# AlessioSam/LADiff

Hardware: AMD Instinct MI355X
Metric: motions/sec (196-frame, 50-step DDIM, bs128) (higher is better)
Workload: dtype f16x3+f32; 1 GPU; headline:ddim50_cfg7.5_b128_f196_c263_humanml3d; prompts_per_gpu=128, global_batch=128, frames=196, scheduler=ddim, denoising_steps=50, parallelism=dp1, loop=persistent pipeline kernel (16-row blocks x 86)

## Files before the change

### include/ladiff_hip_debug.h

```cpp
#ifndef LADIFF_HIP_DEBUG_H
#define LADIFF_HIP_DEBUG_H

#include "ladiff_hip.h"

#ifdef __cplusplus
extern "C" {
#endif

LADIFF_API int ladiff_debug_set_stage_waves(int waves_per_simd);
LADIFF_API int ladiff_debug_set_handoff(int tagged);
LADIFF_API int ladiff_debug_set_stage_plan(int v);
LADIFF_API int ladiff_debug_set_poll_pause(int mask, int len);
LADIFF_API int ladiff_debug_set_stage_delay(int mask, int len);
LADIFF_API int ladiff_debug_set_pacing(int eighths, int mask);
LADIFF_API int ladiff_debug_set_xcd_local(int on);
LADIFF_API int ladiff_debug_set_decoder_fusion(int on);
LADIFF_API int ladiff_debug_set_mlp_variant(int v);

LADIFF_API int ladiff_debug_set_loop_thresholds(int look_ahead_from, int small_upto);
LADIFF_API int ladiff_debug_set_graph_epoch_rule(int on);
LADIFF_API int ladiff_debug_graph_instantiations(void);

#ifdef LADIFF_STAMPS
LADIFF_API void ladiff_debug_set_stamps(unsigned long long* p);
LADIFF_API void ladiff_debug_set_sys_stamps(unsigned long long* p);
LADIFF_API void ladiff_debug_set_probe(int v);
#endif

#ifdef __cplusplus
}
#endif
#endif
```

### ladiff_amd/_lib.py

```python
import ctypes
import os
from ctypes import c_char_p, c_double, c_float, c_int, c_size_t, c_uint64, c_void_p

import numpy as np
import torch

_HERE = os.path.dirname(os.path.abspath(__file__))
LIB_PATH = os.path.join(_HERE, "libladiff_hip.so")

MAX_LATENTS = 8
MAX_FRAMES = 224
COEF_STRIDE = 8
COEF_K_NOISE, COEF_K_M = 5, 6
ACT = {"none": 0, "relu": 1, "gelu": 2, "silu": 3, "qgelu": 4, "lrelu": 5}


class LadiffHipError(RuntimeError):
    pass


SPLIT_MODES = ("f16x3", "bf16x3", "split")


def is_split(precision):
# ... 72 lines not shown
    "ladiff_debug_set_stage_delay": (c_int, [c_int, c_int]),
    "ladiff_debug_set_pacing": (c_int, [c_int, c_int]),
    "ladiff_debug_set_loop_thresholds": (c_int, [c_int, c_int]),
    "ladiff_debug_set_graph_epoch_rule": (c_int, [c_int]),
    "ladiff_debug_graph_instantiations": (c_int, []),
    "ladiff_sampler_set_fault": (c_int, [c_void_p, c_int, c_int]),
    "ladiff_sampler_set_noise_generator": (c_int, [c_void_p, c_uint64, ctypes.c_uint32, c_int]),
    "ladiff_noise_fill": (c_int, [c_uint64, ctypes.c_uint32, c_int, c_int, c_int, c_int, c_void_p, c_void_p]),
    "ladiff_reverse_workspace_bytes": (c_size_t, [c_int, c_int, c_int, c_int]),
    "ladiff_diffusion_reverse": (c_int, [c_void_p, c_void_p, c_void_p, c_uint64, c_void_p, c_void_p, c_void_p, c_void_p, c_void_p,
                                         c_void_p, c_void_p, c_void_p, c_float, c_float, c_int, c_int, c_int, c_int, c_int,
                                         c_void_p, c_void_p, c_size_t, c_int, c_void_p]),
    "ladiff_diffusion_reverse_prompts": (c_int, [c_void_p, c_void_p, c_void_p, c_uint64, c_void_p, c_void_p, c_void_p, c_void_p, c_void_p,
                                                 c_void_p, c_void_p, c_void_p, c_float, c_float, c_int, c_int, c_int, c_int, c_int,
                                                 c_void_p, c_void_p, c_size_t, c_int, c_void_p, c_void_p, c_void_p, c_int, c_void_p]),
    "ladiff_diffusion_reverse_multistep": (c_int, [c_void_p, c_void_p, c_void_p, c_uint64, c_void_p, c_void_p, c_void_p, c_void_p, c_void_p,
                                                   c_void_p, c_void_p, c_void_p, c_float, c_float, c_int, c_int, c_int, c_int, c_int,
                                                   c_void_p, c_void_p, c_size_t, c_int, c_void_p, c_void_p, c_void_p, c_int, c_void_p,
                                                   c_void_p]),
    "ladiff_diffusion_reverse_from": (c_int, [c_void_p, c_void_p, c_void_p, c_uint64, c_void_p, c_void_p, c_void_p, c_void_p, c_void_p,
                                              c_void_p, c_void_p, c_void_p, c_float, c_float, c_int, c_int, c_int, c_int, c_int,
                                              c_void_p, c_void_p, c_size_t, c_int, c_void_p, c_void_p, c_void_p, c_int, c_void_p,
                                              c_void_p, c_void_p, c_int, c_void_p]),
    "ladiff_diffusion_reverse_record": (c_int, [c_void_p, c_void_p, c_void_p, c_uint64, c_void_p, c_void_p, c_void_p, c_void_p, c_void_p,
                                                c_void_p, c_void_p, c_void_p, c_float, c_float, c_int, c_int, c_int, c_int, c_int,
                                                c_void_p, c_void_p, c_size_t, c_int, c_void_p, c_void_p, c_void_p, c_int, c_void_p,
                                                c_void_p, c_void_p, c_int, c_void_p, c_void_p, c_void_p]),
    "ladiff_noise_fill_prompts": (c_int, [c_void_p, c_void_p, c_int, c_int, c_int, c_int, c_void_p, c_void_p]),
    "ladiff_encoder_num_params": (c_int, []),
    "ladiff_encoder_param_name": (c_char_p, [c_int]),
    "ladiff_encoder_workspace_bytes": (c_size_t, [c_int, c_int, c_int, c_int]),
    "ladiff_vae_encode": (c_int, [c_void_p, c_void_p, c_void_p, c_void_p, c_void_p, c_void_p, c_int, c_int, c_int, c_int,
                                  c_void_p, c_void_p, c_void_p, c_void_p, c_size_t, c_void_p]),
    "ladiff_vae_encode_dvae": (c_int, [c_void_p, c_void_p, c_void_p, c_void_p, c_void_p, c_void_p, c_int, c_int, c_int, c_int,
                                       c_void_p, c_void_p, c_void_p, c_void_p, c_size_t, c_void_p, c_void_p, c_int, c_void_p]),
    "ladiff_vae_losses_workspace_bytes": (c_size_t, [c_int, c_int, c_int, c_int, c_int]),
    "ladiff_vae_losses": (c_int, [c_void_p, c_void_p, c_void_p, c_void_p, c_void_p, c_void_p, c_int, c_int, c_int, c_int, c_int,
                                  c_double, c_double, c_double, c_void_p, c_void_p, c_void_p, c_size_t, c_void_p]),
    "ladiff_denoiser_forward_timesteps_workspace_bytes": (c_size_t, [c_int, c_int]),
    "ladiff_denoiser_forward_timesteps": (c_int, [c_void_p, c_void_p, c_void_p, c_int, c_void_p, c_void_p, c_int, c_int, c_void_p, c_void_p,
                                                  c_void_p, c_size_t, c_void_p]),
    "ladiff_q_sample": (c_int, [c_void_p, c_void_p, c_void_p, c_int, c_void_p, c_int, c_uint64, ctypes.c_uint32, c_void_p, c_void_p, c_int,
                                c_int, c_void_p]),
    "ladiff_diffusion_losses_workspace_bytes": (c_size_t, [ctypes.c_int64]),
    "ladiff_diffusion_losses": (c_int, [c_void_p, c_void_p, ctypes.c_int64, c_double, c_void_p, c_void_p, c_void_p, c_size_t, c_void_p]),
    "ladiff_clip_num_params": (c_int, []),
    "ladiff_clip_param_name": (c_char_p, [c_int]),
    "ladiff_clip_workspace_bytes": (c_size_t, [c_int, c_int]),
    "ladiff_clip_text_encode": (c_int, [c_void_p, c_void_p, c_int, c_int, c_void_p, c_int, c_int, c_int, c_void_p, c_void_p,
                                        c_size_t, c_void_p]),
    "ladiff_clip_workspace_bytes_ragged": (c_size_t, [c_int, c_int]),
    "ladiff_clip_text_encode_ragged": (c_int, [c_void_p, c_void_p, c_int, c_int, c_void_p, c_int, c_int, c_int, c_void_p, c_void_p,
                                               c_void_p, c_int, c_void_p, c_void_p, c_size_t, c_void_p]),
    "ladiff_t2m_movement_num_params": (c_int, []),
    "ladiff_t2m_movement_param_name": (c_char_p, [c_int]),
    "ladiff_t2m_motion_num_params": (c_int, []),
    "ladiff_t2m_motion_param_name": (c_char_p, [c_int]),
    "ladiff_t2m_text_num_params": (c_int, []),
    "ladiff_t2m_text_param_name": (c_char_p, [c_int]),
    "ladiff_t2m_movement_workspace_bytes": (c_size_t, [c_int, c_int, c_int]),
    "ladiff_t2m_motion_workspace_bytes": (c_size_t, [c_int, c_int]),
    "ladiff_t2m_text_workspace_bytes": (c_size_t, [c_int, c_int]),
    "ladiff_t2m_movement_encode": (c_int, [c_void_p, c_void_p, c_int, c_int, c_int, c_int, c_void_p, c_void_p, c_size_t,
                                           c_void_p]),
    "ladiff_t2m_motion_encode": (c_int, [c_void_p, c_void_p, c_void_p, c_int, c_int, c_void_p, c_void_p, c_size_t, c_void_p]),
    "ladiff_t2m_text_encode": (c_int, [c_void_p, c_void_p, c_void_p, c_void_p, c_int, c_int, c_void_p, c_void_p, c_size_t,
                                       c_void_p]),
    "ladiff_feats2joints": (c_int, [c_void_p, c_void_p, c_void_p, c_int, c_int, c_int, c_int, c_void_p, c_void_p]),
    "ladiff_joints2feats": (c_int, [c_void_p, c_void_p, c_int, c_int, c_int, c_void_p, c_float, c_void_p, c_void_p, c_void_p, c_void_p]),
    "ladiff_joint_ape_ave": (c_int, [c_void_p, c_void_p, c_void_p, c_void_p, c_int, c_int, c_int, c_void_p, c_float, c_void_p, c_void_p,
                                     c_void_p]),
    "ladiff_joint_mr": (c_int, [c_void_p, c_void_p, c_void_p, c_int, c_int, c_int, c_void_p, c_void_p, c_void_p]),
    "ladiff_render_workspace_bytes": (c_size_t, [c_int]),
    "ladiff_render_motion": (c_int, [c_void_p, c_void_p, c_int, c_int, c_int, c_void_p, c_int, c_int, c_int, c_int, c_void_p, c_int, c_void_p,
                                     c_size_t, c_void_p]),
    "ladiff_decoder_workspace_bytes": (c_size_t, [c_int, c_int, c_int, c_int]),
    "ladiff_vae_decode": (c_int, [c_void_p, c_void_p, c_void_p, c_void_p, c_void_p, c_int, c_int, c_int, c_int, c_void_p,
                                  c_void_p, c_size_t, c_void_p]),
    "ladiff_debug_set_stage_waves": (c_int, [c_int]),
    "ladiff_debug_set_handoff": (c_int, [c_int]),
    "ladiff_debug_set_xcd_local": (c_int, [c_int]),
    "ladiff_debug_set_decoder_fusion": (c_int, [c_int]),
    "ladiff_debug_set_mlp_variant": (c_int, [c_int]),
    "ladiff_reverse_plan": (c_int, [c_int, c_int, c_void_p, c_int, c_int, c_int, c_int, c_void_p, c_void_p]),
    "ladiff_decoder_graph_create": (c_int, [ctypes.POINTER(c_void_p)]),
    "ladiff_decoder_graph_destroy": (c_int, [c_void_p]),
    "ladiff_vae_decode_graphed": (c_int, [c_void_p, c_void_p, c_void_p, c_uint64, c_void_p, c_void_p, c_void_p, c_void_p, c_int, c_int, c_int,
                                          c_int, c_int, c_void_p, c_void_p, c_size_t, c_void_p]),
    "ladiff_vae_decode_ragged": (c_int, [c_void_p, c_void_p, c_void_p, c_void_p, c_void_p, c_void_p, c_int, c_int, c_int, c_int,
                                         c_int, c_void_p, c_void_p, c_size_t, c_void_p]),
    "ladiff_vae_decode_att_maps": (c_int, [c_void_p, c_void_p, c_void_p, c_void_p, c_void_p, c_void_p, c_int, c_int, c_int, c_int,
                                           c_int, c_void_p, c_void_p, c_void_p, c_size_t, c_void_p]),
}

EXPORTS = tuple(_SIGNATURES)
_lib = None
LIB_PATH_BF16 = os.path.join(_HERE, "libladiff_hip_bf16.so")


def select_split_format(fmt):
    global LIB_PATH, _lib
    if fmt not in ("fp16", "bf16"):
        raise ValueError(f'split format must be "fp16" or "bf16", got {fmt!r}')
    path = LIB_PATH_BF16 if fmt == "bf16" else os.path.join(_HERE, "libladiff_hip.so")
    if _lib is not None and path != LIB_PATH:
        raise LadiffHipError("select_split_format() after the library has been used: weight tables of the other format exist")
    LIB_PATH = path


def lib():
    global _lib
    if _lib is None:
        if not os.path.exists(LIB_PATH):
            raise LadiffHipError(f"{LIB_PATH} not found: build it with `python -m ladiff_amd.build` "
                                 "(the HIP library is the only implementation of this path; there is no CPU fallback)")
        cdll = ctypes.CDLL(LIB_PATH)
        for name, (res, args) in _SIGNATURES.items():
            fn = getattr(cdll, name)
            fn.restype, fn.argtypes = res, args
        _lib = cdll
    return _lib


def check(rc):
    if rc != 0:
        raise LadiffHipError(f"libladiff_hip: {lib().ladiff_error_string(rc).decode()} (code {rc})")


def ptr(t, dtype=torch.float32):
    if t is None:
        return None
    if not t.is_cuda:
        raise LadiffHipError("libladiff_hip works on GPU tensors only; got a CPU tensor (no CPU fallback exists)")
    if t.dtype != dtype:
        raise LadiffHipError(f"expected {dtype}, got {t.dtype}")
    if not t.is_contiguous():
        raise LadiffHipError("expected a contiguous tensor")
    return t.data_ptr()


def stream_ptr():
    return torch.cuda.current_stream().cuda_stream


def param_names(kind):
    l = lib()
    n = getattr(l, f"ladiff_{kind}_num_params")()
    return [getattr(l, f"ladiff_{kind}_param_name")(i).decode() for i in range(n)]


class WeightTable:
    _next_generation = 1

    def __init__(self, kind, tensors, n_names=None, no_split=(), pad_rows=None):
        self.generation = WeightTable._next_generation
        WeightTable._next_generation += 1
        names = param_names(kind)
        if n_names is not None:
            names = names[:n_names]
        self.no_split = set(no_split)
        self.pad_rows = dict(pad_rows or {})
        self.names = names
        self.tensors = []
        for n in names:
            if n not in tensors:
                raise LadiffHipError(f"missing weight {n}")
# ... 107 lines not shown
```

### ladiff_amd/build.py

```python
import os
import subprocess
import sys
from concurrent.futures import ThreadPoolExecutor

HERE = os.path.dirname(os.path.abspath(__file__))
CSRC = os.path.join(HERE, "csrc")
OBJ = os.path.join(HERE, "csrc", "build")
LIB = os.path.join(HERE, "libladiff_hip.so")
SOURCES = ["gemm.hip", "gemm_big.hip", "gemm_kr.hip", "gemm_rowln.hip", "rowops.hip", "attention.hip", "qkv_attn.hip", "systolic.hip", "systolic_plan.hip", "linear_ca.hip", "dec_cross.hip", "dec_mlp.hip", "dec_post.hip", "dec_qkv_attn.hip", "feats2joints.hip", "joints2feats.hip", "joint_metrics.hip", "render.hip", "vae_losses.hip", "denoiser.hip", "diffusion_stage.hip", "decoder.hip", "encoder.hip", "clip.hip", "evaluator.hip", "reverse.hip", "api.hip"]
FLAGS = ["--offload-arch=gfx950", "-O3", "-std=c++17", "-fPIC", "-fvisibility=hidden", "-Wall", "-Wno-unused-function"]


def _hipcc():
    for c in (os.environ.get("HIPCC"), "/opt/rocm/bin/hipcc", "hipcc"):
        if c and (os.path.isabs(c) and os.path.exists(c) or not os.path.isabs(c)):
            return c
    raise RuntimeError("hipcc not found")


def _stale(target, deps):
    if not os.path.exists(target):
        return True
    t = os.path.getmtime(target)
    return any(os.path.getmtime(d) > t for d in deps)


def stamps_lib(level=1):
    return LIB.replace(".so", "_stamps.so" if int(level) == 1 else f"_stamps{int(level)}.so")


def diag_lib():
    return LIB.replace(".so", "_diag.so")


def build(force=False, verbose=False, stamps=False, tag=None, defines=(), only=None):
    obj, lib, flags = OBJ, LIB, list(FLAGS)
    if tag:
        obj, lib = OBJ + "_" + tag, LIB.replace(".so", f"_{tag}.so")
        flags += ["-D" + d for d in defines]
    if stamps:
        lvl = os.environ.get("LADIFF_STAMPS_LEVEL", "1")
        obj, lib = OBJ + "_stamps" + (lvl if lvl != "1" else ""), stamps_lib(lvl)
        flags.append("-DLADIFF_STAMPS=" + lvl)
    os.makedirs(obj, exist_ok=True)
    headers = [os.path.join(CSRC, f) for f in os.listdir(CSRC) if f.endswith(".h")]
    headers += [os.path.join(os.path.dirname(HERE), "include", h) for h in ("ladiff_hip.h", "ladiff_hip_debug.h")]
    hipcc = _hipcc()
    jobs = []
    objdir = {src: (obj if only is None or src in only else OBJ) for src in SOURCES}
    for src in SOURCES:
        s = os.path.join(CSRC, src)
        o = os.path.join(objdir[src], src.replace(".hip", ".o"))
        if objdir[src] == obj and (force or _stale(o, [s] + headers)):
            jobs.append([hipcc, *flags, "-c", s, "-o", o])

    def run(cmd):
        if verbose:
            print(" ".join(cmd), flush=True)
        r = subprocess.run(cmd, capture_output=True, text=True)
        if r.returncode != 0:
            raise RuntimeError(f"hipcc failed: {' '.join(cmd)}\n{r.stdout}\n{r.stderr}")
        return r.stderr

    with ThreadPoolExecutor(max_workers=4) as ex:
        for err in ex.map(run, jobs):
            if verbose and err.strip():
                print(err)
    objs = [os.path.join(objdir[s], s.replace(".hip", ".o")) for s in SOURCES]
    if force or jobs or _stale(lib, objs + [os.path.join(CSRC, "exports.map")]):
        run([hipcc, "--offload-arch=gfx950", "-shared", "-fPIC", "-fvisibility=hidden", "-Wl,--version-script=" + os.path.join(CSRC, "exports.map"),
             "-o", lib, *objs])
    return lib


def build_all(force=False, verbose=False):
    lib = build(force=force, verbose=verbose)
    build(force=force, verbose=verbose, tag="bf16", defines=["LADIFF_SPLIT_BF16"])
    build(force=force, verbose=verbose, tag="diag", defines=["LADIFF_TAG_BITS=4", "LADIFF_SELFCHECK"], only=("systolic.hip",))
    return lib


if __name__ == "__main__":
    _tag = next((a.split("=", 1)[1] for a in sys.argv if a.startswith("--tag=")), None)
    _defs = [a[2:] for a in sys.argv if a.startswith("-D")]
    if "--all" in sys.argv:
        print(build_all(force="--force" in sys.argv, verbose=True))
    else:
        print(build(force="--force" in sys.argv, verbose=True, stamps="--stamps" in sys.argv, tag=_tag, defines=_defs))
```

### ladiff_amd/csrc/api.hip

```cpp
#include <algorithm>
#include <cstdlib>
#include <cstring>
#include <vector>

#include "model.h"
#include "sampler.h"
#include "../../include/ladiff_hip_debug.h"

using namespace ladiff;

namespace {

inline hipStream_t S(ladiff_stream_t s) { return reinterpret_cast<hipStream_t>(s); }

bool all_set(const float* const* w, size_t n) {
    if (w == nullptr) return false;
    for (size_t i = 0; i < n; ++i)
        if (w[i] == nullptr) return false;
    return true;
}
template <class W>
bool load_weights(W& dst, const float* const* ptrs) {
    if (!all_set(ptrs, sizeof(W) / sizeof(const float*))) return false;
    std::memcpy(&dst, ptrs, sizeof(W));
// ... 207 lines not shown
int ladiff_init_latents(const float* noise, const int32_t* counts, float sigma, float* latents, int B, int T,
                        ladiff_stream_t stream) {
    LADIFF_CHECK_ARG(noise && latents && B > 0 && T > 0);
    return launch_init_latents(noise, counts, sigma, latents, B, T, S(stream));
}
int ladiff_init_latents_from(const float* z0, const float* noise, const uint64_t* seeds, const uint32_t* prompt_index, const int32_t* counts,
                             const float* coef, const int32_t* starts, int first_step, float* latents, int B, int T, ladiff_stream_t stream) {
    LADIFF_CHECK_ARG(z0 && coef && latents && B > 0 && T > 0 && first_step >= 0);
    LADIFF_CHECK_ARG(noise != nullptr || seeds != nullptr);
    LADIFF_CHECK_ARG(prompt_index == nullptr || seeds != nullptr);
    if ((reinterpret_cast<uintptr_t>(z0) & 15) || (reinterpret_cast<uintptr_t>(noise) & 15) || (reinterpret_cast<uintptr_t>(latents) & 15) ||
        (reinterpret_cast<uintptr_t>(seeds) & 7) || (reinterpret_cast<uintptr_t>(prompt_index) & 3) || (reinterpret_cast<uintptr_t>(starts) & 3))
        return LADIFF_ERR_SHAPE;
    const NoiseGen gen = noise == nullptr ? NoiseGen{0u, 0u, 0u, 1, reinterpret_cast<const unsigned long long*>(seeds), prompt_index}
                                          : NoiseGen{0u, 0u, 0u, 0};
    return launch_init_latents_from(z0, noise, gen, counts, coef, starts, first_step, latents, B, T, nullptr, S(stream));
}
int ladiff_finalize_latents(const float* latents, const int32_t* counts, float* z, int B, int T, ladiff_stream_t stream) {
    LADIFF_CHECK_ARG(latents && z && B > 0 && T > 0);
    return launch_finalize_latents(latents, counts, z, B, T, S(stream));
}

int ladiff_sampler_create(void** sampler) {
    LADIFF_CHECK_ARG(sampler);
    *sampler = new Sampler();
    return 0;
}
int ladiff_sampler_destroy(void* sampler) {
    Sampler* sp = reinterpret_cast<Sampler*>(sampler);
    if (sp == nullptr) return 0;
    (void)hipDeviceSynchronize();
    sp->drain_retired();
    if (sp->exec) (void)hipGraphExecDestroy(sp->exec);
    if (sp->setup) (void)hipGraphExecDestroy(sp->setup);
    if (sp->ev0) (void)hipEventDestroy(sp->ev0);
    if (sp->ev1) (void)hipEventDestroy(sp->ev1);
    for (hipEvent_t e : sp->wev) (void)hipEventDestroy(e);
    sp->cap.destroy();
    delete sp;
    return 0;
}

int ladiff_reverse_plan(int B, int T, const int32_t* h_counts, int masked, int loop_mode, int f16x3, int cfg, int* rows_per_block, int* n_blocks) {
    LADIFF_CHECK_ARG(B >= 1 && T >= 1 && T <= LADIFF_MAX_LATENTS && loop_mode >= 1 && loop_mode <= 3 && rows_per_block && n_blocks);
    if (!cfg && masked && h_counts == nullptr) return LADIFF_ERR_UNSUPPORTED;
    std::vector<unsigned char> plan;
    int mr = 2, nb = 0;
    choose_plan(B, T, h_counts, masked != 0, loop_mode, f16x3 != 0, plan, &mr, &nb, cfg != 0);
    *rows_per_block = 16 * mr; *n_blocks = nb;
    return 0;
}

int ladiff_debug_set_stage_waves(int waves_per_simd) {
    LADIFF_CHECK_ARG(waves_per_simd == 1 || waves_per_simd == 2);
    g_loop.waves16 = waves_per_simd;
    return 0;
}

int ladiff_debug_set_handoff(int tagged) {
    LADIFF_CHECK_ARG(tagged == 0 || tagged == 1);
    g_loop.handoff = tagged;
    return 0;
}

int ladiff_debug_set_mlp_variant(int v) {
#ifdef LADIFF_STAMPS
    LADIFF_CHECK_ARG((v >= 0 && v <= 3) || (v >= 11 && v <= 17) || (v >= 21 && v <= 26));
#else
    LADIFF_CHECK_ARG(v >= 0 && v <= 3);
#endif
    g_dec.mlp_variant = v;
    return 0;
}

int ladiff_debug_set_decoder_fusion(int on) {
    LADIFF_CHECK_ARG(on >= 0 && on <= 254 && (on & 3) != 3 && (on & 48) != 48);
    g_dec.post_off = (on & 128) ? 1 : 0;
    g_dec.out_cross = (on & 64) ? 0 : 1;
    g_dec.fused_mlp = on & 3;
    g_dec.small_rows_path = (on & 4) ? 0 : 1;
    g_dec.final_split = (on & 8) ? 0 : 1;
    g_dec.fused_attn = (on & 16) ? 0 : (on & 32) ? 2 : 1;
    return 0;
}

int ladiff_debug_set_stage_plan(int v) {
    LADIFF_CHECK_ARG(v >= 0 && v <= 1);
    g_loop.stage_plan = v;
    return 0;
}

int ladiff_debug_set_poll_pause(int mask, int len) {
    LADIFF_CHECK_ARG(mask >= 0 && mask <= 255 && len >= 0 && len <= 64);
    g_loop.poll_pause = mask | (len << 8);
    return 0;
}

int ladiff_debug_set_pacing(int eighths, int mask) {
    if (eighths == -1) { g_loop.pace = -1; return 0; }
    LADIFF_CHECK_ARG(eighths >= 0 && eighths <= 8 && mask >= 0 && mask <= 255);
    g_loop.pace = eighths | (mask << 8);
    return 0;
}

int ladiff_debug_set_stage_delay(int mask, int len) {
    LADIFF_CHECK_ARG(mask >= -1 && mask <= 255 && len >= 0 && len <= 64);
    g_loop.stage_delay = mask < 0 ? -1 : (mask | (len << 8));
    return 0;
}

int ladiff_debug_set_loop_thresholds(int look_ahead_from, int small_upto) {
    LADIFF_CHECK_ARG(look_ahead_from >= -1 && small_upto >= -1);
    g_loop.look_ahead_from = look_ahead_from;
    g_loop.small_upto = small_upto;
    return 0;
}

int ladiff_debug_set_graph_epoch_rule(int on) {
    LADIFF_CHECK_ARG(on == 0 || on == 1);
    g_graph_epoch_rule = on;
    return 0;
}

int ladiff_debug_graph_instantiations(void) { return g_graph_instantiations.load(); }

int ladiff_debug_set_xcd_local(int on) {
    LADIFF_CHECK_ARG(on >= 0 && on <= 2);
    g_loop.xcd_local = on;
    return 0;
}

int ladiff_sampler_set_loop(void* sampler, int mode) {
    Sampler* sp = reinterpret_cast<Sampler*>(sampler);
    LADIFF_CHECK_ARG(sp != nullptr && mode >= 0 && mode <= 3);
    sp->loop = mode != 0;
    sp->loop_mode = mode;
    return 0;
}

int ladiff_sampler_loop_ms(void* sampler, float* ms) {
    Sampler* sp = reinterpret_cast<Sampler*>(sampler);
    LADIFF_CHECK_ARG(sp != nullptr && ms != nullptr && sp->ev1 != nullptr);
    LADIFF_HIP(hipEventSynchronize(sp->ev1));
    LADIFF_HIP(hipEventElapsedTime(ms, sp->ev0, sp->ev1));
    return 0;
}

int ladiff_sampler_set_window_timing(void* sampler, int on) {
    Sampler* sp = reinterpret_cast<Sampler*>(sampler);
    LADIFF_CHECK_ARG(sp != nullptr);
    sp->time_windows = on != 0;
    return 0;
}

int ladiff_sampler_window_ms(void* sampler, float* loop_ms_sum, int* n_windows) {
    Sampler* sp = reinterpret_cast<Sampler*>(sampler);
    LADIFF_CHECK_ARG(sp != nullptr && loop_ms_sum != nullptr && n_windows != nullptr);
    float sum = 0.f;
    for (int i = 0; i < sp->n_windows; ++i) {
        float ms = 0.f;
        LADIFF_HIP(hipEventSynchronize(sp->wev[2 * i + 1]));
        LADIFF_HIP(hipEventElapsedTime(&ms, sp->wev[2 * i], sp->wev[2 * i + 1]));
        sum += ms;
    }
    *loop_ms_sum = sum; *n_windows = sp->n_windows;
    return 0;
// ... 487 lines not shown
```

### ladiff_amd/csrc/denoiser.hip

```cpp
#include "model.h"

namespace ladiff {

static std::vector<std::string> block_prefixes(const char* root) {
    std::vector<std::string> v;
    for (int i = 0; i < NSKIP; ++i) v.push_back(std::string(root) + ".input_blocks." + std::to_string(i));
    v.push_back(std::string(root) + ".middle_block");
    for (int i = 0; i < NSKIP; ++i) v.push_back(std::string(root) + ".output_blocks." + std::to_string(i));
    return v;
}
static void wb(std::vector<std::string>& v, const std::string& p) { v.push_back(p + ".weight"); v.push_back(p + ".bias"); }
static void mha_names(std::vector<std::string>& v, const std::string& p) {
    v.push_back(p + ".in_proj_weight"); v.push_back(p + ".in_proj_bias"); wb(v, p + ".out_proj");
}
static void styl_names(std::vector<std::string>& v, const std::string& p) {
    wb(v, p + ".emb_layers.1"); wb(v, p + ".norm"); wb(v, p + ".out_layers.2");
}

const std::vector<std::string>& denoiser_param_names() {
    static const std::vector<std::string> names = [] {
        std::vector<std::string> v;
        wb(v, "time_embedding.linear_1"); wb(v, "time_embedding.linear_2"); wb(v, "emb_proj.1");
        v.push_back("query_pos.pe"); v.push_back("mem_pos.pe");
        wb(v, "encoder.norm");
// ... 27 lines not shown
        return v;
    }();
    return names;
}

const std::vector<std::string>& encoder_param_names() {
    static const std::vector<std::string> names = [] {
        std::vector<std::string> v;
        v.push_back("global_motion_token"); v.push_back("query_pos_encoder.pe");
        for (const auto& p : block_prefixes("encoder")) {
            mha_names(v, p + ".self_attn");
            wb(v, p + ".linear1"); wb(v, p + ".linear2");
            wb(v, p + ".norm1"); wb(v, p + ".norm2");
        }
        for (int i = 0; i < NSKIP; ++i) wb(v, "encoder.linear_blocks." + std::to_string(i));
        wb(v, "encoder.norm"); wb(v, "skel_embedding");
        return v;
    }();
    return names;
}

int denoiser_time_tables(const DenoiserW& w, const float* sinus, int n, float* tables, float* ws, size_t ws_floats,
                         hipStream_t s) {
    const DenTimeWs t = den_time_layout(ws, n);
    if (ws_floats < t.total) return LADIFF_ERR_WORKSPACE;
    float *h1 = t.h1, *temb = t.temb, *semb = t.semb;
    LADIFF_TRY(launch_gemm(lin(sinus, TEXT_DIM, w.time1, h1, D, n, D, TEXT_DIM, ACT_SILU), s));
    LADIFF_TRY(launch_gemm(lin(h1, D, w.time2, temb, D, n, D, D), s));
    LADIFF_TRY(launch_silu(temb, semb, (size_t)n * D, s));
    for (int l = 0; l < NL; ++l) {
        const DenLayerW& L = w.layer[l];
        float* base = tables + (size_t)l * DEN_LAYER_STRIDE;
        LADIFF_TRY(launch_gemm(lin(semb, D, L.ca_proj.emb, base + DEN_OFF_CA_MOD, DEN_STEP_STRIDE, n, 2 * D, D), s));
        LADIFF_TRY(launch_gemm(lin(semb, D, L.ffn_proj.emb, base + DEN_OFF_FFN_MOD, DEN_STEP_STRIDE, n, 2 * D, D), s));
        LinearW kvw{L.sa_attn.in_w + (size_t)D * D, L.sa_attn.in_b + D};
        LADIFF_TRY(launch_gemm(lin(temb, D, kvw, base + DEN_OFF_TIME_KV, DEN_STEP_STRIDE, n, 2 * D, D), s));
    }
    return 0;
}

static int denoiser_text_cache_general(const DenoiserW& w, const float* text, int B2, int N, float* cache, float* ws, size_t ws_floats,
                                       hipStream_t s) {
    const int R = B2 * N;
    const DenTextWs t = den_text_layout(ws, B2, 1, N);
    if (ws_floats < t.total) return LADIFF_ERR_WORKSPACE;
    const DenTextCache c = den_text_cache_layout(cache, B2, 1, N);
    float *rl = t.rl, *tn = t.tn, *key = t.key, *val = t.val, *tproj = c.tproj, *tkv = c.tkv, *catt = c.catt;
    LADIFF_TRY(launch_relu(text, rl, (size_t)R * TEXT_DIM, s));
    LADIFF_TRY(launch_gemm(lin(rl, TEXT_DIM, w.emb_proj, tproj, D, R, D, TEXT_DIM), s));
    for (int l = 0; l < NL; ++l) {
        const DenLayerW& L = w.layer[l];
        LinearW kvw{L.sa_attn.in_w + (size_t)D * D, L.sa_attn.in_b + D};
        LADIFF_TRY(launch_gemm(lin(tproj, D, kvw, tkv + (size_t)l * R * 2 * D, 2 * D, R, 2 * D, D), s));
        LADIFF_TRY(launch_layernorm(tproj, L.ca_text_norm.g, L.ca_text_norm.b, tn, R, s));
        LADIFF_TRY(launch_gemm(lin(tn, D, L.ca_key, key, D, R, D, D), s));
        LADIFF_TRY(launch_gemm(lin(tn, D, L.ca_value, val, D, R, D, D), s));
        LADIFF_TRY(launch_lca_kv(key, val, B2, N, catt + (size_t)l * B2 * H * DH * DH, s));
    }
    return 0;
}

int denoiser_text_static(const DenoiserW& w, const float* text, int B2, float* cache, float* ws, size_t ws_floats, hipStream_t s) {
    const DenTextWs t = den_text_layout(ws, B2, 0, 1);
    if (ws_floats < t.total) return LADIFF_ERR_WORKSPACE;
    const DenTextCache c = den_text_cache_layout(cache, B2, 0, 1);
    float *rl = t.rl, *tn = t.tn, *tproj = c.tproj, *tkv = c.tkv, *nval = c.nval;
    LADIFF_TRY(launch_relu(text, rl, (size_t)B2 * TEXT_DIM, s));
    LADIFF_TRY(launch_gemm(lin(rl, TEXT_DIM, w.emb_proj, tproj, D, B2, D, TEXT_DIM), s));
    GemmArgs kv[NL], val[NL];
    RowBatch ln;
    for (int l = 0; l < NL; ++l) {
        const DenLayerW& L = w.layer[l];
        LinearW kvw{L.sa_attn.in_w + (size_t)D * D, L.sa_attn.in_b + D};
        kv[l] = lin(tproj, D, kvw, tkv + (size_t)l * B2 * 2 * D, 2 * D, B2, 2 * D, D);
        ln.a[l] = tproj; ln.g[l] = L.ca_text_norm.g; ln.b[l] = L.ca_text_norm.b; ln.y[l] = tn + (size_t)l * B2 * D;
        val[l] = lin(tn + (size_t)l * B2 * D, D, L.ca_value, nval + (size_t)l * B2 * D, D, B2, D, D);
        val[l].ln_g = L.ca_proj.norm.g; val[l].ln_b = L.ca_proj.norm.b;
    }
    LADIFF_TRY(launch_gemm_batch(kv, NL, s));
    LADIFF_TRY(launch_layernorm_batch(ln, NL, B2, s));
    return launch_gemm_batch(val, NL, s);
}

int denoiser_ctab(const DenoiserW& w, const float* tables_lo, int n, float* cache, int B2, float* u, size_t u_floats, hipStream_t s,
                  const DenoiserW* wsp) {
    const int R = B2 + 1;
    const size_t u_all = den_text_layout(nullptr, B2, n, 1).u_floats;
    if (u_floats < u_all / NL) return LADIFF_ERR_WORKSPACE;
    const DenTextCache c = den_text_cache_layout(cache, B2, n, 1);
    const float* nval = c.nval;
    float* ctab = c.ctab;
    if (u_floats >= u_all) {
        RowBatch rb;
        GemmArgs g[NL];
        for (int l = 0; l < NL; ++l) {
            const DenLayerW& L = w.layer[l];
            float* ul = u + (size_t)l * n * R * D;
            rb.a[l] = nval + (size_t)l * B2 * D; rb.g[l] = L.ca_proj.norm.b;
            rb.b[l] = tables_lo + (size_t)l * DEN_LAYER_STRIDE + DEN_OFF_CA_MOD; rb.y[l] = ul;
            g[l] = lin(ul, D, L.ca_proj.out, ctab + (size_t)l * n * R * D, D, n * R, D, D);
            if (wsp != nullptr) { g[l].W = wsp->layer[l].ca_proj.out.w; g[l].split = 1; }
        }
        LADIFF_TRY(launch_ca_table_input_batch(rb, NL, DEN_STEP_STRIDE, n, B2, s, wsp != nullptr ? 1 : 0));
        return launch_gemm_batch(g, NL, s);
    }
    for (int l = 0; l < NL; ++l) {
        const DenLayerW& L = w.layer[l];
        LADIFF_TRY(launch_ca_table_input(nval + (size_t)l * B2 * D, L.ca_proj.norm.b, tables_lo + (size_t)l * DEN_LAYER_STRIDE + DEN_OFF_CA_MOD,
                                         DEN_STEP_STRIDE, n, B2, u, s));
        LADIFF_TRY(launch_gemm(lin(u, D, L.ca_proj.out, ctab + (size_t)l * n * R * D, D, n * R, D, D), s));
    }
    return 0;
}

int denoiser_text_cache(const DenoiserW& w, const float* text, int B2, const float* tables, int n, float* cache,
                        float* ws, size_t ws_floats, hipStream_t s, int ntxt) {
    if (ntxt > 1) return denoiser_text_cache_general(w, text, B2, ntxt, cache, ws, ws_floats, s);
    const DenTextWs t = den_text_layout(ws, B2, n, 1);
    if (ws_floats < t.total) return LADIFF_ERR_WORKSPACE;
    LADIFF_TRY(denoiser_text_static(w, text, B2, cache, ws, ws_floats, s));
    return denoiser_ctab(w, tables, n, cache, B2, t.u, t.u_floats, s, nullptr);
}

int linear_cross_attention(const DenoiserW& w, int layer, const float* x, const float* xf, const float* emb, const int32_t* counts,
                           int B, int T, int N, float* out, float* ws, size_t ws_floats, hipStream_t s) {
    if (layer < 0 || layer >= NL || T < 1 || T > LADIFF_MAX_LATENTS || N < 1) return LADIFF_ERR_SHAPE;
    const LcaWs a = lca_layout(ws, B, T, N);
    if (ws_floats < a.total) return LADIFF_ERR_WORKSPACE;
    const DenLayerW& L = w.layer[layer];
    const int R = B * N, M = B * T;
    float *tn = a.tn, *key = a.key, *val = a.val, *catt = a.catt, *xn = a.xn, *q = a.q, *semb = a.semb, *mod = a.mod;
    LADIFF_TRY(launch_layernorm(xf, L.ca_text_norm.g, L.ca_text_norm.b, tn, R, s));
    LADIFF_TRY(launch_gemm(lin(tn, D, L.ca_key, key, D, R, D, D), s));
    LADIFF_TRY(launch_gemm(lin(tn, D, L.ca_value, val, D, R, D, D), s));
    LADIFF_TRY(launch_lca_kv(key, val, B, N, catt, s));
    LADIFF_TRY(launch_layernorm(x, L.ca_norm.g, L.ca_norm.b, xn, M, s));
    LADIFF_TRY(launch_gemm(lin(xn, D, L.ca_query, q, D, M, D, D), s));
    LADIFF_TRY(launch_silu(emb, semb, (size_t)B * D, s));
    LADIFF_TRY(launch_gemm(lin(semb, D, L.ca_proj.emb, mod, 2 * D, B, 2 * D, D), s));
    LADIFF_TRY(launch_lca_apply(q, catt, counts, B, 0, B, T, mod, 0, 2 * D, nullptr, L.ca_proj.norm.g, L.ca_proj.norm.b, xn, s));
    GemmArgs g = lin(xn, D, L.ca_proj.out, out, D, M, D, D);
    g.res = x; g.ldres = D;
    return launch_gemm(g, s);
}


int denoiser_forward(const DenoiserW& w, const DenoiserW* wsp, const float* tables, const int32_t* d_step, const float* cache,
                     int n_steps, const float* sample, int Bs, int dup, int T, const int32_t* counts, float* eps, float* ws,
                     size_t ws_floats, hipStream_t s, int b_lo, int b_n, int loop_mode, int ntxt, const int32_t* d_base,
                     const float* dctab) {
    const int B2 = Bs * dup;
    const bool per_sample = d_step == nullptr;
    if (per_sample && (dctab == nullptr || ntxt != 1 || loop_mode)) return LADIFF_ERR_ARG;
    if (b_n < 0) { b_lo = 0; b_n = B2; }
    const int M = b_n * T;
    if (T < 1 || T > LADIFF_MAX_LATENTS || b_lo < 0 || b_lo + b_n > B2) return LADIFF_ERR_SHAPE;
    if (M == 0) return 0;
    DenForwardWs a = den_forward_layout(ws, (size_t)M);
    if (ws_floats < a.total) return LADIFF_ERR_WORKSPACE;
    eps += (size_t)b_lo * T * D;
    const bool sp = wsp != nullptr;
    const Seq c{sp, M, s};
    const DenoiserW& wm = mfma_table(w, wsp);
    Twin P[4], SK[NSKIP];
    pair_up(sp, a.P, a.Ps, P); pair_up(sp, a.SK, a.SKs, SK);
    float *qkv = a.qkv, *att = a.att, *hid = a.hid, *part = a.part;
    const Twin hid_x = operand_only(sp, hid);
    const float* tkv = den_cache_tkv(cache, B2, ntxt);
    const float* ctab = den_cache_ctab(cache, B2, ntxt);
    const int R = B2 + 1;
    auto gemm = [&](Twin x, int K, const LinearW& W, Twin y, int ldy, int N, int act = ACT_NONE, const float* res = nullptr) {
        return launch_gemm_kr(proj_kr(c, x, K, W, y, ldy, N, act, res), s);
    };

// ... 83 lines not shown
```

### ladiff_amd/csrc/kernels.h

```cpp
#pragma once
#include "common.h"
#include "noise_gen.h"

namespace ladiff {

enum RedMode : int { RED_PLAIN = 0, RED_LN = 1, RED_LN_ADD = 2, RED_LN_MOD = 3 };
struct RedArgs {
    const float* P = nullptr;
    const float* bias = nullptr; const float* res = nullptr;
    const float* g = nullptr; const float* b = nullptr;
    const float* tab = nullptr;
    const int32_t* d_step = nullptr;
    const int32_t* counts = nullptr;
    float* out = nullptr; float* outs = nullptr;
    const int32_t* d_base = nullptr;
    const float* g2 = nullptr; const float* b2 = nullptr;
    size_t plane = 0;
    int S = 1, mode = RED_PLAIN, tab_step_stride = 0, Bs = 1, T = 1, pad_row = 0, b_off = 0, M = 0;
};
int launch_reduce_rows(const RedArgs& a, hipStream_t s, bool per_sample = false);
int launch_split_rows(const float* x, float* y, int R, int K, hipStream_t s);
int launch_gather_rows(const float* src, const int32_t* index, int n_rows, int row_floats, float* dst, hipStream_t s);
int launch_split_range_stats(const float* const* xs, const int64_t* counts, int n, int64_t max_count, unsigned long long* stats,
                             hipStream_t s);
int launch_layernorm(const float* x, const float* g, const float* b, float* y, int M, hipStream_t s);
constexpr int DEC_PREP_MAX = 9;
struct DecCrossPrepBatch { const float* kv[DEC_PREP_MAX]; const float* wq[DEC_PREP_MAX]; const float* bq[DEC_PREP_MAX];
                           const float* wo[DEC_PREP_MAX]; float* gu[DEC_PREP_MAX]; };
constexpr int ROW_BATCH_MAX = 9;
struct RowBatch { const float* a[ROW_BATCH_MAX]; const float* g[ROW_BATCH_MAX]; const float* b[ROW_BATCH_MAX]; float* y[ROW_BATCH_MAX]; };
int launch_layernorm_batch(const RowBatch& rb, int n, int M, hipStream_t s);
int launch_ca_table_input_batch(const RowBatch& rb, int n_layers, int step_stride, int n, int B2, hipStream_t s, int split_out = 0);
int launch_ca_table_input(const float* nval, const float* beta, const float* mod, int step_stride, int n, int B2, float* u,
                          hipStream_t s);
int launch_add_pe(const float* sample, const float* pe, int Bs, int b_off, int b_n, int T, float* x, float* xs, hipStream_t s);
int launch_broadcast_pe(const float* pe, int B, int F, float* x, float* xs, hipStream_t s);
int launch_broadcast_pe_ragged(const float* pe, const int32_t* row_off, int B, int F, int F_out, float* x, float* xs, int32_t* row_out,
                               hipStream_t s);
int launch_relu(const float* x, float* y, size_t n, hipStream_t s);
int launch_pad_rows(const float* src, const float* srcb, float* dst, float* dstb, int C, int Np, hipStream_t s);
int launch_zero_fill(float* x, size_t n, hipStream_t s);
int launch_silu(const float* x, float* y, size_t n, hipStream_t s);
int launch_sinusoid(const int64_t* t, int n, float* out, hipStream_t s);
struct StepEnd {
    const float *coef, *noise;
    NoiseGen gen;
    float g; const float* gs;
    int cfg;
    float* x0_prev;
    bool edit; const int32_t* starts; int first_step;
    float *traj_x, *traj_x0; const int32_t* traj_counts;
    bool record() const { return traj_x != nullptr || traj_x0 != nullptr; }
};
int launch_traj_zero_pad(float* traj, const int32_t* counts, int first, int n, int B, int T, hipStream_t s);
int launch_cfg_step(const float* eps, float* lat, const int32_t* d_step, const StepEnd& e, int B, int T, hipStream_t s);
int launch_advance(int32_t* d_step, hipStream_t s);
int launch_step_tail(float* x, float* xs, const float* ng, const float* nb, float* lat, int32_t* d_step, const float* pe, const StepEnd& e,
                     int B, int T, hipStream_t s);
int launch_noise_fill(const NoiseGen& gen, int step0, int n, int B, int T, float* out, hipStream_t s);
int launch_init_latents(const float* noise, const int32_t* counts, float sigma, float* lat, int B, int T, hipStream_t s);
int launch_init_latents_gen(const NoiseGen& gen, const int32_t* counts, float sigma, float* lat, int B, int T, hipStream_t s);
int launch_init_latents_from(const float* z0, const float* noise, const NoiseGen& gen, const int32_t* counts, const float* coef,
                             const int32_t* starts, int first_step, float* lat, int B, int T, int32_t* d_step, hipStream_t s);
int launch_finalize_latents(const float* lat, const int32_t* counts, float* z, int B, int T, hipStream_t s, const unsigned* status = nullptr);

int launch_dec_qkv_attn(const float* xs, const float* w, const float* bias, const int32_t* lengths, const int32_t* row_off, float* out,
                        int B, int F, int split_out, hipStream_t s);
int launch_scatter_feats(const float* tmp, int ldt, int C, int M, int F, const int32_t* row_len, const int32_t* row_map, float* feats,
                         hipStream_t s);
int launch_pad_cols(const float* x, float* y, int R, int C, int Cp, hipStream_t s);
int launch_dvae_pad_cols(const float* x, const int32_t* slot, const float* values, int n, float* y, int B, int F, int C, int Cp,
                         hipStream_t s);
int launch_encoder_assemble(const float* token, const float* emb, const float* pe, const int32_t* lengths,
                            const int32_t* counts, int B, int F, int T, float* x, float* xs, uint32_t* keybits, hipStream_t s);
int launch_encoder_finalize(const float* out, const float* eps, const int32_t* counts, int B, int T, int S, float* mu, float* sd,
                            float* latent, hipStream_t s);

int launch_lca_kv(const float* key, const float* value, int B, int N, float* att, hipStream_t s);
int launch_lca_apply(const float* q, const float* att, const int32_t* counts, int Bs, int b_off, int b_n, int T, const float* mod,
                     int step_stride, int sample_stride, const int32_t* d_step, const float* g, const float* be, float* u,
                     hipStream_t s);
int launch_denoiser_self_attention_general(const float* qkv, const float* text_kv, int N, const float* tables, int kv_off,
                                           int step_stride, const int32_t* d_step, const int32_t* counts, int Bs, int b_off,
                                           int b_n, int T, float* out, hipStream_t s);

int launch_decoder_cross_prep(const DecCrossPrepBatch& pb, int n, int B, int T, hipStream_t s);
int launch_decoder_out_cross(const float* att_s, const float* x0, const float* wo_s, const float* bo, const float* g1, const float* b1,
                             const float* bo_c, const float* g2, const float* b2, const int32_t* counts, int B, int F, int T,
                             const float* gu_ws, float* y, float* ys, hipStream_t s, const int32_t* row_off);
int launch_decoder_cross_apply(const float* x, const float* bo, const float* g2, const float* b2, const int32_t* counts, int B, int F,
                               int T, const float* gu_ws, float* y, float* ys, hipStream_t s, const int32_t* row_off = nullptr,
                               const float* g1 = nullptr, const float* b1 = nullptr);
int launch_decoder_cross_maps(const float* x, const int32_t* counts, const int32_t* lengths, int B, int F, int T, const float* gu_ws,
                              float* maps, hipStream_t s, const int32_t* row_off, const float* g1, const float* b1);

int launch_feats2joints(const float* feats, const float* mean, const float* stdv, int B, int F, int C, int J, float* joints,
                        hipStream_t s);

int launch_joints2feats(const float* joints, const int32_t* h_lengths, int B, int L, const float* tgt, float feet_thre, const float* mean,
                        const float* stdv, float* feats, hipStream_t s);

size_t render_ws_bytes(int B);
int launch_render_motion(const float* joints, const int32_t* h_lengths, int B, int L, int J, const ladiff_render_params& P, int mode,
                         int n_poses, int H, int W, void* out, int out_is_float, float* ws, size_t ws_bytes, hipStream_t s);

int launch_joint_ape_ave(const float* rst, const float* ref, const int32_t* lengths, int B, int F, int J, const int32_t* part_idx,
                         float factor, float* seq_rows, double* acc, hipStream_t s);
int launch_joint_mr(const float* rst, const float* ref, int B, int F, int J, float* seq_rows, double* acc, hipStream_t s);

int launch_vae_losses(const float* m_rst, const float* m_ref, size_t n_feat, const float* j_rst, const float* j_ref, size_t n_joint,
                      const float* mu, const float* sd, size_t n_lat, double l_rec, double l_joint, double l_kl, double* part, int blocks,
                      double* batch, double* acc, hipStream_t s);

int launch_denoiser_self_attention(const float* qkv, const float* text_kv, const float* tables, int kv_off,
                                   int step_stride, const int32_t* d_step, const int32_t* counts, int Bs, int b_off,
                                   int b_n, int T, float* out, int split_out, hipStream_t s);
int launch_decoder_self_attention(const float* qkv, const int32_t* lengths, const uint32_t* keybits, float* out, int B, int F,
// ... 10 lines not shown
```

### ladiff_amd/csrc/model.h

```cpp
#pragma once
#include <atomic>
#include "graph_key.h"
#include "seq.h"
#include "systolic_plan.h"
#include "workspace.h"

namespace ladiff {

int denoiser_time_tables(const DenoiserW& w, const float* sinus, int n, float* tables, float* ws, size_t ws_floats, hipStream_t s);
int denoiser_text_cache(const DenoiserW& w, const float* text, int B2, const float* tables, int n_steps, float* cache,
                        float* ws, size_t ws_floats, hipStream_t s, int ntxt = 1);
int denoiser_forward(const DenoiserW& w, const DenoiserW* w_split, const float* tables, const int32_t* d_step,
                     const float* cache, int n_steps, const float* sample, int Bs, int dup, int T, const int32_t* counts, float* eps, float* ws,
                     size_t ws_floats, hipStream_t s, int b_lo = 0, int b_n = -1, int loop_mode = 0, int ntxt = 1,
                     const int32_t* d_base = nullptr, const float* dctab = nullptr);
int denoiser_text_static(const DenoiserW& w, const float* text, int B2, float* cache, float* ws, size_t ws_floats, hipStream_t s);
int denoiser_ctab(const DenoiserW& w, const float* tables_lo, int n, float* cache, int B2, float* u, size_t u_floats, hipStream_t s,
                  const DenoiserW* w_split = nullptr);
int linear_cross_attention(const DenoiserW& w, int layer, const float* x, const float* xf, const float* emb, const int32_t* counts,
                           int B, int T, int N, float* out, float* ws, size_t ws_floats, hipStream_t s);

int denoiser_forward_timesteps(const DenoiserW& w, const DenoiserW* w_split, const float* text, const int64_t* timesteps, const float* sample,
                               int B2, int T, const int32_t* counts, float* eps, float* ws, size_t ws_floats, hipStream_t s);
int launch_q_sample(const float* z, const int64_t* ts, const float* acp, int n_train, const int32_t* counts, const NoiseGen& gen, float* noise,
                    float* noisy, int B, int T, hipStream_t s);
int launch_diffusion_losses(const float* pred, const float* noise, size_t n, double lambda_inst, double* part, int blocks, double* batch,
                            double* acc, hipStream_t s);

struct Sampler;
int diffusion_reverse(Sampler* sp, const DenoiserW& w, const DenoiserW* w_split, const ReverseArgs& a);

struct DecSwitchAtoms {
    std::atomic<int> fused_mlp{1}, small_rows_path{1}, final_split{1}, out_cross{1}, fused_attn{1}, mlp_variant{0}, post_off{0};
    DecSwitches snapshot() const { return {fused_mlp, small_rows_path, final_split, out_cross, fused_attn, mlp_variant, post_off}; }
};
extern DecSwitchAtoms g_dec;
int dec_mlp_prepare();
int dec_qkv_attn_prepare();
int dec_cross_prepare();
int dec_mlp_min_rows();
int vae_decode(const DecoderW& w, const DecoderW* w_split, const float* z, const int32_t* lengths, const int32_t* counts,
               const int32_t* row_off, int R, int B, int F, int T, int C, float* feats, float* ws, size_t ws_floats, hipStream_t s, const DecSwitches& sw,
               float* att_maps = nullptr);

int launch_dec_mlp(const float* xs, const float* x, const float* w1, const float* b1, const float* w2, const float* b2, const float* g3,
                   const float* be3, const float* g4, const float* be4, float* y, float* ys, int M, hipStream_t s, int variant);

struct DecPostArgs {
    const float* att;
    const float* x0;
    const float* wo;
    const float *bo, *g1, *be1;
    const float *gu, *cc;
    const float *bo_c, *g2, *be2;
    const int32_t *counts, *row_off;
    const float *w1, *b1, *w2, *b2, *g3, *be3, *g4, *be4;
    float *y, *ys;
    int B, F, T, M;
};
int dec_post_prepare();
int launch_dec_post_gu(float* guws, size_t gu_layer, int n, int B, int T, hipStream_t s);
int launch_dec_post(const DecPostArgs& a, hipStream_t s);

int vae_encode(const EncoderW& w, const EncoderW* w_split, const float* features, const int32_t* lengths,
               const int32_t* counts, const float* eps, int B, int F, int T, int C, float* mu, float* sd, float* latent, float* ws,
               size_t ws_floats, hipStream_t s, const int32_t* slot = nullptr, const float* values = nullptr, int n_values = 0);

#ifdef LADIFF_STAMPS
extern unsigned long long* g_sys_stamps;
extern int g_sys_probe;
#endif
bool sys_supported(int B, int T, int cfg, bool split);
int sys_reset_status(float* ws, hipStream_t s);
int sys_build_stages(const DenoiserW& W, const DenoiserW& WS, float* ws, int MR, int NB, std::vector<unsigned char>& host);
int launch_systolic_loop(const DenoiserW& W, float* ws, const float* tables, const float* tkv, const float* ctab, int n_ctab, float* lat,
                         const int32_t* counts, const StepEnd& e, int B, int T, int step_lo, int n, int fp32, int MR, int NB, hipStream_t s,
                         int fault_wg, unsigned long long timeout_ticks);

int launch_qkv_attention(const float* x, const float* w, const float* bias, const float* text_kv, const float* tables,
                         int kv_off, int step_stride, const int32_t* d_step, const int32_t* counts, int Bs, int b_off,
                         int b_n, int T, float* out, hipStream_t s);

int clip_text_encode(const ClipW& w, const ClipW* w_split, int n_layers, int vocab, const int64_t* ids, int B, int S, int L,
                     float* out, float* ws, size_t ws_floats, hipStream_t s, const int32_t* seq_len = nullptr,
                     const int32_t* row_off = nullptr, const int32_t* row_seq = nullptr, int total_rows = 0);

const std::vector<std::string>& t2m_move_param_names();
const std::vector<std::string>& t2m_motion_param_names();
const std::vector<std::string>& t2m_text_param_names();
int t2m_movement_encode(const float* const* w, const float* feats, int ld, int B, int F, int Cin, float* out, float* ws,
                        size_t ws_floats, hipStream_t s);
int t2m_motion_encode(const float* const* w, const float* mov, const int32_t* m_lens, int B, int T, float* out, float* ws,
                      size_t ws_floats, hipStream_t s);
int t2m_text_encode(const float* const* w, const float* word_embs, const float* pos_onehot, const int32_t* cap_lens, int B, int L,
                    float* out, float* ws, size_t ws_floats, hipStream_t s);

}
```

Baseline: 11440 motions/s.

## Fuse cross-attention modulation table input build and projection GEMM into one kernel

Adds a fused kernel that computes the SiLU-modulated cross-attention table input (norm value scaled and shifted per step), splits it to hi/lo f16 fragments in shared memory, and multiplies by the split output projection weights with bias in a single double-buffered pass across all layers. It replaces the previous two-phase path that wrote the intermediate u buffer to global memory and then ran a batched GEMM. It is the default route when split weights are available, with a debug switch to fall back. The cost is a fixed grid of 256/NL workgroups per layer at one block per CU, which may underuse the GPU when the table is small.

```diff
diff --git a/include/ladiff_hip_debug.h b/include/ladiff_hip_debug.h
--- a/include/ladiff_hip_debug.h
+++ b/include/ladiff_hip_debug.h
@@ -15,6 +15,10 @@
 LADIFF_API int ladiff_debug_set_pacing(int eighths, int mask);
 LADIFF_API int ladiff_debug_set_xcd_local(int on);
 LADIFF_API int ladiff_debug_set_decoder_fusion(int on);
+LADIFF_API int ladiff_debug_set_ctab_route(int fused);
+LADIFF_API int ladiff_debug_ctab_window(const float* const* w, const float* const* w_split, const float* text_emb , int B2,
+                                        const float* tables, int lo, int n_steps, float* cache, void* ws, size_t ws_bytes,
+                                        ladiff_stream_t stream);
 LADIFF_API int ladiff_debug_set_mlp_variant(int v);
 
 LADIFF_API int ladiff_debug_set_loop_thresholds(int look_ahead_from, int small_upto);
diff --git a/ladiff_amd/_lib.py b/ladiff_amd/_lib.py
--- a/ladiff_amd/_lib.py
+++ b/ladiff_amd/_lib.py
@@ -178,6 +178,8 @@
     "ladiff_debug_set_xcd_local": (c_int, [c_int]),
     "ladiff_debug_set_decoder_fusion": (c_int, [c_int]),
     "ladiff_debug_set_mlp_variant": (c_int, [c_int]),
+    "ladiff_debug_set_ctab_route": (c_int, [c_int]),
+    "ladiff_debug_ctab_window": (c_int, [c_void_p, c_void_p, c_void_p, c_int, c_void_p, c_int, c_int, c_void_p, c_void_p, c_size_t, c_void_p]),
     "ladiff_reverse_plan": (c_int, [c_int, c_int, c_void_p, c_int, c_int, c_int, c_int, c_void_p, c_void_p]),
     "ladiff_decoder_graph_create": (c_int, [ctypes.POINTER(c_void_p)]),
     "ladiff_decoder_graph_destroy": (c_int, [c_void_p]),
diff --git a/ladiff_amd/build.py b/ladiff_amd/build.py
--- a/ladiff_amd/build.py
+++ b/ladiff_amd/build.py
@@ -7,7 +7,7 @@
 CSRC = os.path.join(HERE, "csrc")
 OBJ = os.path.join(HERE, "csrc", "build")
 LIB = os.path.join(HERE, "libladiff_hip.so")
-SOURCES = ["gemm.hip", "gemm_big.hip", "gemm_kr.hip", "gemm_rowln.hip", "rowops.hip", "attention.hip", "qkv_attn.hip", "systolic.hip", "systolic_plan.hip", "linear_ca.hip", "dec_cross.hip", "dec_mlp.hip", "dec_post.hip", "dec_qkv_attn.hip", "feats2joints.hip", "joints2feats.hip", "joint_metrics.hip", "render.hip", "vae_losses.hip", "denoiser.hip", "diffusion_stage.hip", "decoder.hip", "encoder.hip", "clip.hip", "evaluator.hip", "reverse.hip", "api.hip"]
+SOURCES = ["gemm.hip", "gemm_big.hip", "gemm_kr.hip", "gemm_rowln.hip", "rowops.hip", "ctab.hip", "attention.hip", "qkv_attn.hip", "systolic.hip", "systolic_plan.hip", "linear_ca.hip", "dec_cross.hip", "dec_mlp.hip", "dec_post.hip", "dec_qkv_attn.hip", "feats2joints.hip", "joints2feats.hip", "joint_metrics.hip", "render.hip", "vae_losses.hip", "denoiser.hip", "diffusion_stage.hip", "decoder.hip", "encoder.hip", "clip.hip", "evaluator.hip", "reverse.hip", "api.hip"]
 FLAGS = ["--offload-arch=gfx950", "-O3", "-std=c++17", "-fPIC", "-fvisibility=hidden", "-Wall", "-Wno-unused-function"]
 
 
diff --git a/ladiff_amd/csrc/api.hip b/ladiff_amd/csrc/api.hip
--- a/ladiff_amd/csrc/api.hip
+++ b/ladiff_amd/csrc/api.hip
@@ -313,6 +313,22 @@
     g_dec.final_split = (on & 8) ? 0 : 1;
     g_dec.fused_attn = (on & 16) ? 0 : (on & 32) ? 2 : 1;
     return 0;
+}
+
+int ladiff_debug_set_ctab_route(int fused) {
+    LADIFF_CHECK_ARG(fused == 0 || fused == 1);
+    g_ctab_route = fused;
+    return 0;
+}
+
+int ladiff_debug_ctab_window(const float* const* w, const float* const* w_split, const float* text_emb, int B2, const float* tables, int lo,
+                             int n_steps, float* cache, void* ws, size_t ws_bytes, ladiff_stream_t stream) {
+    DenoiserW W, WS;
+    LADIFF_CHECK_ARG(load_weights(W, w) && load_weights(WS, w_split) && text_emb && tables && cache && ws && B2 > 0 && lo >= 0 && n_steps > 0);
+    if (ws_bytes < ladiff_denoiser_workspace_bytes(B2, 1, n_steps, 1)) return LADIFF_ERR_WORKSPACE;
+    const DenTextWs t = den_text_layout((float*)ws, B2, n_steps, 1);
+    LADIFF_TRY(denoiser_text_static(W, text_emb, B2, cache, (float*)ws, ws_bytes / sizeof(float), S(stream)));
+    return denoiser_ctab(W, tables + (size_t)lo * DEN_STEP_STRIDE, n_steps, cache, B2, t.u, t.u_floats, S(stream), &WS);
 }
 
 int ladiff_debug_set_stage_plan(int v) {
diff --git a/ladiff_amd/csrc/ctab.hip b/ladiff_amd/csrc/ctab.hip
--- /dev/null
+++ b/ladiff_amd/csrc/ctab.hip
@@ -0,0 +1,102 @@
+#include "kernels.h"
+#include "tile_mma.h"
+
+namespace ladiff {
+
+namespace {
+constexpr int CT_ROWS = 32;
+constexpr int CT_TILE = CT_ROWS * 1024;
+constexpr int CT_WGS = 256 / NL;
+}
+
+__global__ __launch_bounds__(512, 1) void ctab_fused_kernel(const CtabArgs p, int step_stride, int B2, int M) {
+    __shared__ __attribute__((aligned(1024))) char tile[2][CT_TILE];
+    const int layer = blockIdx.y, tid = threadIdx.x, lane = tid & 63, frow = lane & 15, fk = lane >> 4;
+    const int wave = __builtin_amdgcn_readfirstlane(tid >> 6);
+    const int ntiles = (M + 15) / 16;
+    const int r0 = 16 * (int)((long long)blockIdx.x * ntiles / CT_WGS);
+    const int r1e = 16 * (int)((long long)(blockIdx.x + 1) * ntiles / CT_WGS), r1 = r1e < M ? r1e : M;
+    if (r0 >= r1) return;
+    const float* __restrict__ nval = p.nval[layer]; const float* __restrict__ beta = p.beta[layer]; const float* __restrict__ mod = p.mod[layer];
+    float* __restrict__ out = p.out[layer];
+    const int R = B2 + 1, kc = 32 * wave + 8 * fk;
+
+    struct Raw { f32x4 v[2], sc[2], sh[2]; };
+    auto request = [&](int rb, int i, Raw& q) {
+        int r = rb + 16 * i + frow;
+        r = r < r1 ? r : r1 - 1;
+        const int step = r / R, b = r - step * R;
+        const float* m = mod + (size_t)step * step_stride + kc;
+        const float* v = (b < B2 ? nval + (size_t)b * D : beta) + kc;
+        q.v[0] = ld4(v); q.v[1] = ld4(v + 4);
+        q.sc[0] = ld4(m); q.sc[1] = ld4(m + 4);
+        q.sh[0] = ld4(m + 256); q.sh[1] = ld4(m + 260);
+    };
+    auto build = [&](char* t, int i, const Raw& q) {
+        f32x4 u[2];
+#pragma unroll
+        for (int h = 0; h < 2; ++h)
+#pragma unroll
+            for (int e = 0; e < 4; ++e) u[h][e] = silu(q.v[h][e] * (1.f + q.sc[h][e]) + q.sh[h][e]);
+        s16x8 hi, lo;
+        split8(u[0], u[1], hi, lo);
+        const int row = 16 * i + frow;
+        *reinterpret_cast<s16x8*>(a_slot<4>(t, row, wave >> 1, 4 * (wave & 1) + fk)) = hi;
+        *reinterpret_cast<s16x8*>(a_slot<4>(t, row, wave >> 1, 8 + 4 * (wave & 1) + fk)) = lo;
+    };
+
+    Raw qa, qb;
+    request(r0, 0, qa);
+    request(r0, 1, qb);
+    WFrag<0, 2, 8> wf;
+    load_w<0, 2, 8>(wf, p.w[layer], D, 0, [&](int j) { return 32 * wave + 16 * j; });
+    f32x4 bv[2];
+#pragma unroll
+    for (int j = 0; j < 2; ++j) bv[j] = ld4(p.bias[layer] + 32 * wave + 16 * j + 4 * fk);
+    build(tile[0], 0, qa);
+    build(tile[0], 1, qb);
+    landed();
+    __syncthreads();
+    auto store = [&](int rb, const f32x4 (&acc)[2][2], bool whole) {
+#pragma unroll
+        for (int i = 0; i < 2; ++i) {
+            const int row = rb + 16 * i + frow;
+            if (whole || row < r1) {
+#pragma unroll
+                for (int j = 0; j < 2; ++j) {
+                    f32x4 o;
+#pragma unroll
+                    for (int e = 0; e < 4; ++e) o[e] = (acc[i][j][e] + bv[j][e]) + 0.f;
+                    st4(out + (size_t)row * D + 32 * wave + 16 * j + 4 * fk, o);
+                }
+            }
+        }
+    };
+    int rb = r0, buf = 0;
+    for (; rb + CT_ROWS < r1; rb += CT_ROWS, buf ^= 1) {
+        request(rb + CT_ROWS, 0, qa);
+        f32x4 acc[2][2];
+        zero_acc(acc);
+        mma<0, 4, 2, 8, 2, 2, 1, true>(tile[buf], wf, acc);
+        request(rb + CT_ROWS, 1, qb);
+        store(rb, acc, true);
+        build(tile[buf ^ 1], 0, qa);
+        build(tile[buf ^ 1], 1, qb);
+        asm volatile("s_waitcnt lgkmcnt(0)\n\ts_barrier" ::: "memory");
+    }
+    f32x4 acc[2][2];
+    zero_acc(acc);
+    mma<0, 4, 2, 8, 2, 2, 1, true>(tile[buf], wf, acc);
+    store(rb, acc, false);
+}
+
+int launch_ctab_fused(const CtabArgs& a, int step_stride, int n, int B2, hipStream_t s) {
+    LADIFF_CHECK_ARG(n >= 0 && B2 >= 0 && (long long)n * (B2 + 1) < (1ll << 31) - 64);
+    const int M = n * (B2 + 1);
+    if (M == 0) return 0;
+    hipLaunchKernelGGL(ctab_fused_kernel, dim3(CT_WGS, NL), dim3(512), 0, s, a, step_stride, B2, M);
+    LADIFF_LAUNCH_CHECK();
+    return 0;
+}
+
+}
diff --git a/ladiff_amd/csrc/denoiser.hip b/ladiff_amd/csrc/denoiser.hip
--- a/ladiff_amd/csrc/denoiser.hip
+++ b/ladiff_amd/csrc/denoiser.hip
@@ -133,6 +133,7 @@
     return launch_gemm_batch(val, NL, s);
 }
 
+std::atomic<int> g_ctab_route{1};
 int denoiser_ctab(const DenoiserW& w, const float* tables_lo, int n, float* cache, int B2, float* u, size_t u_floats, hipStream_t s,
                   const DenoiserW* wsp) {
     const int R = B2 + 1;
@@ -141,6 +142,17 @@
     const DenTextCache c = den_text_cache_layout(cache, B2, n, 1);
     const float* nval = c.nval;
     float* ctab = c.ctab;
+    if (u_floats >= u_all && wsp != nullptr && g_ctab_route.load() == 1) {
+        CtabArgs a;
+        for (int l = 0; l < NL; ++l) {
+            const DenLayerW& L = w.layer[l];
+            a.nval[l] = nval + (size_t)l * B2 * D; a.beta[l] = L.ca_proj.norm.b;
+            a.mod[l] = tables_lo + (size_t)l * DEN_LAYER_STRIDE + DEN_OFF_CA_MOD;
+            a.w[l] = wsp->layer[l].ca_proj.out.w; a.bias[l] = L.ca_proj.out.b;
+            a.out[l] = ctab + (size_t)l * n * R * D;
+        }
+        return launch_ctab_fused(a, DEN_STEP_STRIDE, n, B2, s);
+    }
     if (u_floats >= u_all) {
         RowBatch rb;
         GemmArgs g[NL];
diff --git a/ladiff_amd/csrc/kernels.h b/ladiff_amd/csrc/kernels.h
--- a/ladiff_amd/csrc/kernels.h
+++ b/ladiff_amd/csrc/kernels.h
@@ -33,6 +33,8 @@
 int launch_ca_table_input_batch(const RowBatch& rb, int n_layers, int step_stride, int n, int B2, hipStream_t s, int split_out = 0);
 int launch_ca_table_input(const float* nval, const float* beta, const float* mod, int step_stride, int n, int B2, float* u,
                           hipStream_t s);
+struct CtabArgs { const float* nval[NL]; const float* beta[NL]; const float* mod[NL]; const float* w[NL]; const float* bias[NL]; float* out[NL]; };
+int launch_ctab_fused(const CtabArgs& a, int step_stride, int n, int B2, hipStream_t s);
 int launch_add_pe(const float* sample, const float* pe, int Bs, int b_off, int b_n, int T, float* x, float* xs, hipStream_t s);
 int launch_broadcast_pe(const float* pe, int B, int F, float* x, float* xs, hipStream_t s);
 int launch_broadcast_pe_ragged(const float* pe, const int32_t* row_off, int B, int F, int F_out, float* x, float* xs, int32_t* row_out,
diff --git a/ladiff_amd/csrc/model.h b/ladiff_amd/csrc/model.h
--- a/ladiff_amd/csrc/model.h
+++ b/ladiff_amd/csrc/model.h
@@ -17,6 +17,7 @@
 int denoiser_text_static(const DenoiserW& w, const float* text, int B2, float* cache, float* ws, size_t ws_floats, hipStream_t s);
 int denoiser_ctab(const DenoiserW& w, const float* tables_lo, int n, float* cache, int B2, float* u, size_t u_floats, hipStream_t s,
                   const DenoiserW* w_split = nullptr);
+extern std::atomic<int> g_ctab_route;
 int linear_cross_attention(const DenoiserW& w, int layer, const float* x, const float* xf, const float* emb, const int32_t* counts,
                            int B, int T, int N, float* out, float* ws, size_t ws_floats, hipStream_t s);
 
```

After: 11540 motions/s (median of 6 runs). No clear change (+0.8%).
